# gargatik/Seamless-Through-Breaking-Rethinking-Image-Stitching-for-Optimal-Alignment

Measured on AMD Instinct MI355X. Metric: stitched image-pairs/s at 512x512, higher is better.
Workload: dtype f32 (decoder contractions, PatchEmbed's third conv and the C = 128 block tails: exact 3xbf16 split of both operands, 6 products on the bf16 matrix cores, fp32 accumulate -- error vs fp64 0.83x the fp32 MFMA chain's; everything else fp32); 1 GPU; UDIS-D-shaped 512x512 pairs, batch=1, FlowHomoAdpater.forward(type=test_eval); launch=hipGraph replay, pairs_in_flight=3

## Files before the change

seamless-through-breaking-rethinking-image-stitching-for-optimal-alignment_amd/csrc/gemm_split3.h:

```cpp
#pragma once
#include "gemm_common.h"

__global__ __launch_bounds__(256) void split3_pack_kernel(const float* __restrict__ x, __bf16* __restrict__ planes, long long rows, int C,
                                                          long long ldx, long long plane_stride, long long chunk_rows) {
    const long long idx = (long long)blockIdx.x * 256 + threadIdx.x;
    const int groups = C >> 3;
    if (idx >= rows * groups) return;
    const int g4 = (int)(idx & 3);
    const long long t = idx >> 2;
    const long long row = t % rows;
    const int chunk = (int)(t / rows);
    const float4 v0 = *reinterpret_cast<const float4*>(x + row * ldx + chunk * 32 + g4 * 8);
    const float4 v1 = *reinterpret_cast<const float4*>(x + row * ldx + chunk * 32 + g4 * 8 + 4);
    const float v[8] = {v0.x, v0.y, v0.z, v0.w, v1.x, v1.y, v1.z, v1.w};
    bf16x8 h, m, l;
#pragma unroll
    for (int e = 0; e < 8; ++e) {
        __bf16 a, b, c;
        st_split3(v[e], a, b, c);
        h[e] = a; m[e] = b; l[e] = c;
    }
    const long long o = ((long long)chunk * chunk_rows + row) * 32 + g4 * 8;
    *reinterpret_cast<bf16x8*>(planes + o) = h;
    *reinterpret_cast<bf16x8*>(planes + plane_stride + o) = m;
    *reinterpret_cast<bf16x8*>(planes + 2 * plane_stride + o) = l;
}

template <int WM, int WN, int TM, int TN, int STAGES, int KPAR = 1>
__device__ __forceinline__ void conv_gemm_split3_body(const st_gemm_desc& d, const int block_id) {
    static_assert(WM * WN == 4, "4 consumer waves per K half (+ 4 loader waves)");
    static_assert(KPAR == 1 || KPAR == 2, "one or two consumer groups");
    constexpr int BM = WM * TM * 32, BN = WN * TN * 32, ROWS = BM + BN;
    constexpr int PLANE_B = ROWS * 64, STAGE_B = 3 * PLANE_B;
    constexpr int GA = BM / 16, GB = BN / 16;
    static_assert((3 * GA) % 4 == 0 && (3 * GB) % 4 == 0, "pieces divide among the 4 loader waves");
    constexpr int PA = 3 * GA / 4, PB = 3 * GB / 4, PPW = PA + PB;
    static_assert((STAGES - 1) * PPW <= 63 && STAGES >= 3 && STAGES <= 4, "vmcnt immediate");
    extern __shared__ __attribute__((aligned(1024))) float smem[];
    char* const sm = reinterpret_cast<char*>(smem);

    const int tid = threadIdx.x;
    const int lane = tid & 63, wave = __builtin_amdgcn_readfirstlane(tid >> 6);
    const int split = d.split_k > 1 ? d.split_k : 1;
    const int bz = split > 1 ? 0 : blockIdx.z;
    const int kz = split > 1 ? blockIdx.z : 0;

    const int ntm = (d.M + BM - 1) / BM, ntn = (d.N + BN - 1) / BN;
    const int nwg = ntm * ntn;
    int bid = block_id;
    {
        const int q = nwg >> 3, r = nwg & 7, xcd = bid & 7, idx = bid >> 3;
        bid = (xcd < r ? xcd * (q + 1) : r * (q + 1) + (xcd - r) * q) + idx;
    }
    const int tile_n = bid % ntn, tile_m = bid / ntn;
    const int m0 = tile_m * BM, n0 = tile_n * BN;

    const int nkt_all = d.K / 32;
    const int per = (nkt_all + split - 1) / split;
    const int kt0 = kz * per;
    const int ntiles = min(nkt_all, kt0 + per) - kt0;

    if (wave >= 4 * KPAR) {
        const int lw = wave - 4 * KPAR;
        const char* A = reinterpret_cast<const char*>(d.a) + (size_t)bz * d.batch_stride_a * 2;
        const char* A2 = d.a2 ? reinterpret_cast<const char*>(d.a2) + (size_t)bz * d.batch_stride_a * 2 : A;
        const char* Wt = reinterpret_cast<const char*>(d.w) + (size_t)bz * d.batch_stride_w * 2;
        const i32x4 rsrcA = make_rsrc(A, d.a_bytes), rsrcA2 = make_rsrc(A2, d.a_bytes), rsrcW = make_rsrc(Wt, d.w_bytes);
        const int a2c = d.a2 ? d.a2_channels : 0;
        const unsigned lds0 = (unsigned)(size_t)(__attribute__((address_space(3))) char*)sm;
        const unsigned a_plane_b = (unsigned)(d.a_plane_stride * 2), w_plane_b = (unsigned)(d.w_plane_stride * 2);
        const unsigned a_chunk_b = (unsigned)(d.a_rows * 64), w_chunk_b = (unsigned)(d.w_rows * 64);

        int a_row[PA], a_iy0[PA], a_ix0[PA];
        unsigned a_c[PA], voffA[PA], voffB[PB], ldsA[PA], ldsB[PB];
#pragma unroll
        for (int i = 0; i < PA; ++i) {
            const int q = lw * PA + i, plane = q / GA, rg = q % GA;
            const int r = 16 * rg + (lane >> 2), c = (lane & 3) ^ ((r >> 2) & 3);
            const int m = min(m0 + r, d.M - 1);
            const int hw = d.Ho * d.Wo;
            const int b = m / hw, rr = m - b * hw;
            const int oy = rr / d.Wo, ox = rr - oy * d.Wo;
            a_iy0[i] = oy * d.sh - d.ph; a_ix0[i] = ox * d.sw - d.pw;
            a_row[i] = (b * d.H + a_iy0[i]) * d.W + a_ix0[i];
            a_c[i] = (unsigned)plane * a_plane_b + (unsigned)c * 16u;
            ldsA[i] = __builtin_amdgcn_readfirstlane(lds0 + (unsigned)(plane * PLANE_B + rg * 1024));
        }
#pragma unroll
        for (int i = 0; i < PB; ++i) {
            const int q = lw * PB + i, plane = q / GB, rg = q % GB;
            const int r = 16 * rg + (lane >> 2), c = (lane & 3) ^ ((r >> 2) & 3);
            voffB[i] = (unsigned)plane * w_plane_b + (unsigned)min(n0 + r, d.N - 1) * 64u + (unsigned)c * 16u;
            ldsB[i] = __builtin_amdgcn_readfirstlane(lds0 + (unsigned)(plane * PLANE_B + BM * 64 + rg * 1024));
        }
        int i_c0, i_ky, i_kx;
        {
            const int k = kt0 * 32, tap = k / d.Cin;
            i_c0 = k - tap * d.Cin; i_ky = tap / d.kw; i_kx = tap - i_ky * d.kw;
        }
        unsigned soffA = (unsigned)(i_c0 >> 5) * a_chunk_b, soffB = (unsigned)kt0 * w_chunk_b;
        auto set_tap = [&]() {
            const int ty = i_ky * (d.dh > 1 ? d.dh : 1), tx = i_kx * (d.dw > 1 ? d.dw : 1);
            const int tapoff = ty * d.W + tx;
#pragma unroll
            for (int i = 0; i < PA; ++i) {
                const bool ok = (unsigned)(a_iy0[i] + ty) < (unsigned)d.H && (unsigned)(a_ix0[i] + tx) < (unsigned)d.W;
                voffA[i] = ok ? a_c[i] + (unsigned)(a_row[i] + tapoff) * 64u : ST_OOB;
            }
        };
        set_tap();
        auto issue_tile = [&](int stage) {
            const unsigned so = (unsigned)(stage * STAGE_B);
            const bool second = i_c0 < a2c;
#pragma unroll
            for (int i = 0; i < PA; ++i) lds_dma16(second ? rsrcA2 : rsrcA, ldsA[i] + so, voffA[i], soffA);
#pragma unroll
            for (int i = 0; i < PB; ++i) lds_dma16(rsrcW, ldsB[i] + so, voffB[i], soffB);
            soffB += w_chunk_b; soffA += a_chunk_b;
            i_c0 += 32;
            if (i_c0 >= d.Cin) {
                i_c0 = 0; soffA = 0;
                if (++i_kx == d.kw) { i_kx = 0; ++i_ky; }
                set_tap();
            }
        };
        auto wait_tiles = [&](int tiles) {
            if (tiles >= 3) asm volatile("s_waitcnt vmcnt(%0)" ::"n"(3 * PPW) : "memory");
            else if (tiles == 2) asm volatile("s_waitcnt vmcnt(%0)" ::"n"(2 * PPW) : "memory");
            else if (tiles == 1) asm volatile("s_waitcnt vmcnt(%0)" ::"n"(PPW) : "memory");
            else asm volatile("s_waitcnt vmcnt(0)" ::: "memory");
        };
        for (int t = 0; t < STAGES && t < ntiles; ++t) issue_tile(t);
        wait_tiles(min(STAGES - 1, ntiles - 1));
        asm volatile("s_barrier" ::: "memory");
        int stage = 0;
        for (int t = 0; t + 1 < ntiles; ++t) {
            wait_tiles(min(STAGES - 2, ntiles - 2 - t));
            asm volatile("s_barrier" ::: "memory");
            if (t + STAGES < ntiles) issue_tile(stage);
            stage = stage == STAGES - 1 ? 0 : stage + 1;
        }
        return;
    }

    float* __restrict__ C = d.c + (size_t)bz * d.batch_stride_c;
    const int grp = KPAR == 2 ? wave >> 2 : 0, cw = KPAR == 2 ? wave & 3 : wave;
    const int wm = cw / WN, wn = cw % WN;
    const int li = lane & 31, lh = lane >> 5;

    f32x16 acc[TM][TN], tot[TM][TN];
#pragma unroll
    for (int i = 0; i < TM; ++i)
#pragma unroll
        for (int j = 0; j < TN; ++j)
#pragma unroll
            for (int r = 0; r < 16; ++r) { acc[i][j][r] = 0.f; tot[i][j][r] = 0.f; }
    constexpr int KBLK = 8;

    const char* pa[2];
    const char* pb[2];
#pragma unroll
    for (int j = 0; j < 2; ++j) {
        const int ch = (2 * j + lh) ^ ((li >> 2) & 3);
        pa[j] = sm + (wm * TM * 32 + li) * 64 + ch * 16;
        pb[j] = sm + (BM + wn * TN * 32 + li) * 64 + ch * 16;
    }
    if constexpr (KPAR == 2) {
        bf16x8 ga[2][3][TM], gb[2][3][TN];
        const int chg = (2 * grp + lh) ^ ((li >> 2) & 3);
        const char* const qa = sm + (wm * TM * 32 + li) * 64 + chg * 16;
        const char* const qb = sm + (BM + wn * TN * 32 + li) * 64 + chg * 16;
        auto kread = [&](int nbuf, int nstage, int set) {
            const int ra = set == 0 ? 2 : set == 1 ? 0 : 1, rb = set == 0 ? 0 : set == 1 ? 2 : 1;
#pragma unroll
            for (int r = 0; r < TM; ++r) ga[nbuf][ra][r] = *reinterpret_cast<const bf16x8*>(qa + nstage * STAGE_B + ra * PLANE_B + r * 2048);
#pragma unroll
            for (int r = 0; r < TN; ++r) gb[nbuf][rb][r] = *reinterpret_cast<const bf16x8*>(qb + nstage * STAGE_B + rb * PLANE_B + r * 2048);
        };
        auto kprod = [&](int buf, int nbuf, int p, int q, int nstage, int set) {
            const int ra = set == 0 ? 2 : set == 1 ? 0 : 1, rb = set == 0 ? 0 : set == 1 ? 2 : 1;
            constexpr int NM = TM * TN, NR = TM + TN;
            int issued = 0;
#pragma unroll
            for (int i = 0; i < TM; ++i)
#pragma unroll
                for (int jn = 0; jn < TN; ++jn) {
                    acc[i][jn] = __builtin_amdgcn_mfma_f32_32x32x16_bf16(ga[buf][p][i], gb[buf][q][jn], acc[i][jn], 0, 0, 0);
                    if (set >= 0) {
                        const int upto = ((i * TN + jn + 1) * NR + NM - 1) / NM;
#pragma unroll
                        for (int r = 0; r < NR; ++r)
                            if (r >= issued && r < upto) {
                                if (r < TM) ga[nbuf][ra][r] = *reinterpret_cast<const bf16x8*>(qa + nstage * STAGE_B + ra * PLANE_B + r * 2048);
                                else gb[nbuf][rb][r - TM] = *reinterpret_cast<const bf16x8*>(qb + nstage * STAGE_B + rb * PLANE_B + (r - TM) * 2048);
                            }
                        issued = upto;
                    }
                    __builtin_amdgcn_sched_barrier(0);
                }
        };
        constexpr bool EPI_AHEAD2 = TM * TN == 1;
        EpiOperands<TM, TN> eop2;
        if (EPI_AHEAD2 && grp == 0) {
            gemm_epilogue_consts<TM, TN>(d, eop2, n0, wn, li, split);
            gemm_epilogue_load<TM, TN>(d, eop2, m0, n0, wm, wn, li, lh, split);
            __builtin_amdgcn_sched_barrier(0);
        }
        asm volatile("s_barrier" ::: "memory");
        kread(0, 0, 0); kread(0, 0, 1); kread(0, 0, 2);
        __builtin_amdgcn_sched_barrier(0);
        auto kstep = [&](auto more_c, int buf, int nbuf, int s, int t, bool more_rt) {
            constexpr bool MORE = decltype(more_c)::value;
            if (MORE || more_rt) {
                asm volatile("s_waitcnt lgkmcnt(0)\n\ts_barrier" ::: "memory");
                kprod(buf, nbuf, 2, 0, (s + 1) % STAGES, 0); kprod(buf, nbuf, 0, 2, (s + 1) % STAGES, 1); kprod(buf, nbuf, 1, 1, (s + 1) % STAGES, 2);
            } else {
                kprod(buf, nbuf, 2, 0, 0, -1); kprod(buf, nbuf, 0, 2, 0, -1); kprod(buf, nbuf, 1, 1, 0, -1);
            }
            kprod(buf, nbuf, 1, 0, 0, -1); kprod(buf, nbuf, 0, 1, 0, -1); kprod(buf, nbuf, 0, 0, 0, -1);
            if ((t & (KBLK - 1)) == KBLK - 1 && (MORE || more_rt)) {
#pragma unroll
                for (int i = 0; i < TM; ++i)
#pragma unroll
                    for (int j = 0; j < TN; ++j) {
                        tot[i][j] = tot[i][j] + acc[i][j];
#pragma unroll
                        for (int r = 0; r < 16; ++r) acc[i][j][r] = 0.f;
                    }
                __builtin_amdgcn_sched_barrier(0);
            }
        };
        static_assert(STAGES % 2 == 0, "the fragment buffers alternate with the steps: an even ring keeps (stage, buffer) literal in the unrolled turn");
        int tb = 0;
        for (; tb + STAGES < ntiles; tb += STAGES) {
#pragma unroll
            for (int s = 0; s < STAGES; ++s) kstep(st_true{}, s & 1, (s & 1) ^ 1, s, tb + s, true);
        }
#pragma unroll
        for (int s = 0; s < STAGES; ++s)
            if (tb + s < ntiles) kstep(st_false{}, s & 1, (s & 1) ^ 1, s, tb + s, tb + s + 1 < ntiles);
        if (ntiles > KBLK) {
#pragma unroll
            for (int i = 0; i < TM; ++i)
#pragma unroll
                for (int j = 0; j < TN; ++j) acc[i][j] = acc[i][j] + tot[i][j];
        }
        asm volatile("s_waitcnt lgkmcnt(0)\n\ts_barrier" ::: "memory");
        float* const red = reinterpret_cast<float*>(sm) + (size_t)cw * (TM * TN * 16 * 64) + lane;
        if (grp == 1) {
#pragma unroll
            for (int i = 0; i < TM; ++i)
#pragma unroll
                for (int j = 0; j < TN; ++j)
#pragma unroll
                    for (int r = 0; r < 16; ++r) red[((i * TN + j) * 16 + r) * 64] = acc[i][j][r];
        }
        __syncthreads();
        if (grp == 1) return;
#pragma unroll
        for (int i = 0; i < TM; ++i)
#pragma unroll
            for (int j = 0; j < TN; ++j)
#pragma unroll
                for (int r = 0; r < 16; ++r) acc[i][j][r] += red[((i * TN + j) * 16 + r) * 64];
        if (EPI_AHEAD2) gemm_epilogue_store<TM, TN, false, false>(d, C, acc, eop2, m0, n0, wm, wn, li, lh, split, kz);
        else gemm_tile_epilogue<TM, TN>(d, C, acc, m0, n0, wm, wn, li, lh, split, kz);
        return;
    }
    bf16x8 fa[2][3][TM], fb[2][3][TN];
    auto prod = [&](int buf, int p, int q, int nbuf, int nstage, int nj, int set) {
        const int ra = set == 0 ? 2 : set == 1 ? 0 : 1, rb = set == 0 ? 0 : set == 1 ? 2 : 1;
        constexpr int NM = TM * TN, NR = TM + TN;
        int issued = 0;
#pragma unroll
        for (int i = 0; i < TM; ++i)
#pragma unroll
            for (int jn = 0; jn < TN; ++jn) {
                acc[i][jn] = __builtin_amdgcn_mfma_f32_32x32x16_bf16(fa[buf][p][i], fb[buf][q][jn], acc[i][jn], 0, 0, 0);
                if (set >= 0) {
                    const int upto = ((i * TN + jn + 1) * NR + NM - 1) / NM;
#pragma unroll
                    for (int r = 0; r < NR; ++r)
                        if (r >= issued && r < upto) {
                            if (r < TM) fa[nbuf][ra][r] = *reinterpret_cast<const bf16x8*>(pa[nj] + nstage * STAGE_B + ra * PLANE_B + r * 2048);
                            else fb[nbuf][rb][r - TM] = *reinterpret_cast<const bf16x8*>(pb[nj] + nstage * STAGE_B + rb * PLANE_B + (r - TM) * 2048);
                        }
                    issued = upto;
                }
                __builtin_amdgcn_sched_barrier(0);
            }
    };
    auto read_set = [&](int nbuf, int nstage, int nj, int set) {
        const int ra = set == 0 ? 2 : set == 1 ? 0 : 1, rb = set == 0 ? 0 : set == 1 ? 2 : 1;
#pragma unroll
        for (int r = 0; r < TM; ++r) fa[nbuf][ra][r] = *reinterpret_cast<const bf16x8*>(pa[nj] + nstage * STAGE_B + ra * PLANE_B + r * 2048);
#pragma unroll
        for (int r = 0; r < TN; ++r) fb[nbuf][rb][r] = *reinterpret_cast<const bf16x8*>(pb[nj] + nstage * STAGE_B + rb * PLANE_B + r * 2048);
    };

    constexpr bool EPI_AHEAD = TM * TN == 1;
    EpiOperands<TM, TN> eop;
    if (EPI_AHEAD) {
        gemm_epilogue_consts<TM, TN>(d, eop, n0, wn, li, split);
        gemm_epilogue_load<TM, TN>(d, eop, m0, n0, wm, wn, li, lh, split);
        __builtin_amdgcn_sched_barrier(0);
    }

    asm volatile("s_barrier" ::: "memory");
    read_set(0, 0, 0, 0); read_set(0, 0, 0, 1); read_set(0, 0, 0, 2);
    __builtin_amdgcn_sched_barrier(0);
    auto tile_body = [&](auto more_c, int s, int t, bool more_rt) {
        constexpr bool MORE = decltype(more_c)::value;
        prod(0, 2, 0, 1, s, 1, 0); prod(0, 0, 2, 1, s, 1, 1); prod(0, 1, 1, 1, s, 1, 2);
        prod(0, 1, 0, 0, 0, 0, -1); prod(0, 0, 1, 0, 0, 0, -1); prod(0, 0, 0, 0, 0, 0, -1);
        if (MORE || more_rt) {
            asm volatile("s_waitcnt lgkmcnt(0)\n\ts_barrier" ::: "memory");
            prod(1, 2, 0, 0, (s + 1) % STAGES, 0, 0); prod(1, 0, 2, 0, (s + 1) % STAGES, 0, 1); prod(1, 1, 1, 0, (s + 1) % STAGES, 0, 2);
        } else {
            prod(1, 2, 0, 0, 0, 0, -1); prod(1, 0, 2, 0, 0, 0, -1); prod(1, 1, 1, 0, 0, 0, -1);
        }
        prod(1, 1, 0, 0, 0, 0, -1); prod(1, 0, 1, 0, 0, 0, -1); prod(1, 0, 0, 0, 0, 0, -1);
        if ((t & (KBLK - 1)) == KBLK - 1 && (MORE || more_rt)) {
#pragma unroll
            for (int i = 0; i < TM; ++i)
#pragma unroll
                for (int j = 0; j < TN; ++j) {
                    tot[i][j] = tot[i][j] + acc[i][j];
#pragma unroll
                    for (int r = 0; r < 16; ++r) acc[i][j][r] = 0.f;
                }
            __builtin_amdgcn_sched_barrier(0);
        }
    };
    int tb = 0;
    for (; tb + STAGES < ntiles; tb += STAGES) {
#pragma unroll
        for (int s = 0; s < STAGES; ++s) tile_body(st_true{}, s, tb + s, true);
    }
#pragma unroll
    for (int s = 0; s < STAGES; ++s)
        if (tb + s < ntiles) tile_body(st_false{}, s, tb + s, tb + s + 1 < ntiles);
    if (ntiles > KBLK) {
#pragma unroll
        for (int i = 0; i < TM; ++i)
#pragma unroll
            for (int j = 0; j < TN; ++j) acc[i][j] = acc[i][j] + tot[i][j];
    }
    if (EPI_AHEAD) gemm_epilogue_store<TM, TN, false, false>(d, C, acc, eop, m0, n0, wm, wn, li, lh, split, kz);
    else gemm_tile_epilogue<TM, TN>(d, C, acc, m0, n0, wm, wn, li, lh, split, kz);
}

template <bool CT>
__device__ __forceinline__ void conv_gemm_split3_persist_body(const st_gemm_desc& d) {
    constexpr int BM = 64, BN = 64, ROWS = 128, STAGES = 3, WN = 2;
    constexpr int PLANE_B = ROWS * 64, STAGE_B = 3 * PLANE_B, GA = 4, GB = 4, PA = 3, PB = 3, PPW = 6;
    extern __shared__ __attribute__((aligned(1024))) float smem[];
    char* const sm = reinterpret_cast<char*>(smem);
    const int tid = threadIdx.x;
    const int lane = tid & 63, wave = __builtin_amdgcn_readfirstlane(tid >> 6);
    const int bz = blockIdx.z;
    const int ntm = (d.M + BM - 1) / BM, ntn = (d.N + BN - 1) / BN, ntl = ntm * ntn;
    const int G = (int)gridDim.x, w = (int)blockIdx.x;
    const int nmine = (ntl - w + G - 1) / G;
    const int nkt = d.K / 32;
    const int total = nmine * nkt;

    if (wave >= 4) {
        const int lw = wave - 4;
        const char* A = reinterpret_cast<const char*>(d.a) + (size_t)bz * d.batch_stride_a * 2;
        const char* Wt = reinterpret_cast<const char*>(d.w) + (size_t)bz * d.batch_stride_w * 2;
        const i32x4 rsrcA = make_rsrc(A, d.a_bytes), rsrcW = make_rsrc(Wt, d.w_bytes);
        const unsigned lds0 = (unsigned)(size_t)(__attribute__((address_space(3))) char*)sm;
        const unsigned a_plane_b = (unsigned)(d.a_plane_stride * 2), w_plane_b = (unsigned)(d.w_plane_stride * 2);
        const unsigned a_chunk_b = (unsigned)(d.a_rows * 64), w_chunk_b = (unsigned)(d.w_rows * 64);
        int a_row[PA], a_iy0[PA], a_ix0[PA];
        unsigned a_c[PA], voffA[PA], voffB[PB], ldsA[PA], ldsB[PB];
#pragma unroll
        for (int i = 0; i < PA; ++i) {
            const int q = lw * PA + i, plane = q / GA, rg = q % GA;
            ldsA[i] = __builtin_amdgcn_readfirstlane(lds0 + (unsigned)(plane * PLANE_B + rg * 1024));
        }
#pragma unroll
        for (int i = 0; i < PB; ++i) {
            const int q = lw * PB + i, plane = q / GB, rg = q % GB;
            ldsB[i] = __builtin_amdgcn_readfirstlane(lds0 + (unsigned)(plane * PLANE_B + BM * 64 + rg * 1024));
        }
        int i_c0 = 0, i_ky = 0, i_kx = 0, i_kt = 0, i_tile = w;
        unsigned soffA = 0, soffB = 0;
        auto set_tap = [&]() {
            const int ty = i_ky * (d.dh > 1 ? d.dh : 1), tx = i_kx * (d.dw > 1 ? d.dw : 1);
            const int tapoff = ty * d.W + tx;
#pragma unroll
            for (int i = 0; i < PA; ++i) {
                const bool ok = (unsigned)(a_iy0[i] + ty) < (unsigned)d.H && (unsigned)(a_ix0[i] + tx) < (unsigned)d.W;
                voffA[i] = ok ? a_c[i] + (unsigned)(a_row[i] + tapoff) * 64u : ST_OOB;
            }
        };
        auto set_tile = [&](int idx) {
            const int m0 = (idx / ntn) * BM, n0 = (idx % ntn) * BN;
#pragma unroll
            for (int i = 0; i < PA; ++i) {
                const int q = lw * PA + i, plane = q / GA, rg = q % GA;
                const int r = 16 * rg + (lane >> 2), c = (lane & 3) ^ ((r >> 2) & 3);
                const int m = min(m0 + r, d.M - 1);
                const int hw = d.Ho * d.Wo;
                const int b = m / hw, rr = m - b * hw;
                const int oy = rr / d.Wo, ox = rr - oy * d.Wo;
                a_iy0[i] = oy * d.sh - d.ph; a_ix0[i] = ox * d.sw - d.pw;
                a_row[i] = (b * d.H + a_iy0[i]) * d.W + a_ix0[i];
                a_c[i] = (unsigned)plane * a_plane_b + (unsigned)c * 16u;
            }
#pragma unroll
            for (int i = 0; i < PB; ++i) {
                const int q = lw * PB + i, plane = q / GB, rg = q % GB;
                const int r = 16 * rg + (lane >> 2), c = (lane & 3) ^ ((r >> 2) & 3);
                voffB[i] = (unsigned)plane * w_plane_b + (unsigned)min(n0 + r, d.N - 1) * 64u + (unsigned)c * 16u;
            }
            i_c0 = 0; i_ky = 0; i_kx = 0; i_kt = 0; soffA = 0; soffB = 0;
            set_tap();
        };
        set_tile(i_tile);
        auto issue_step = [&](int stage) {
            const unsigned so = (unsigned)(stage * STAGE_B);
            const unsigned sa = __builtin_amdgcn_readfirstlane(soffA), sb = __builtin_amdgcn_readfirstlane(soffB);
#pragma unroll
            for (int i = 0; i < PA; ++i) lds_dma16(rsrcA, ldsA[i] + so, voffA[i], sa);
#pragma unroll
            for (int i = 0; i < PB; ++i) lds_dma16(rsrcW, ldsB[i] + so, voffB[i], sb);
            if (++i_kt == nkt) { i_tile += G; if (i_tile < ntl) set_tile(i_tile); return; }
            soffB += w_chunk_b; soffA += a_chunk_b;
            i_c0 += 32;
            if (i_c0 >= d.Cin) {
                i_c0 = 0; soffA = 0;
                if (++i_kx == d.kw) { i_kx = 0; ++i_ky; }
                set_tap();
            }
        };
        auto wait_tiles = [&](int tiles) {
            if (tiles >= 2) asm volatile("s_waitcnt vmcnt(%0)" ::"n"(2 * PPW) : "memory");
            else if (tiles == 1) asm volatile("s_waitcnt vmcnt(%0)" ::"n"(PPW) : "memory");
            else asm volatile("s_waitcnt vmcnt(0)" ::: "memory");
        };
        for (int t = 0; t < STAGES && t < total; ++t) issue_step(t);
        wait_tiles(min(STAGES - 1, total - 1));
        asm volatile("s_barrier" ::: "memory");
        int stage = 0;
        for (int t = 0; t + 1 < total; ++t) {
            wait_tiles(min(STAGES - 2, total - 2 - t));
            asm volatile("s_barrier" ::: "memory");
            if (t + STAGES < total) issue_step(stage);
            stage = stage == STAGES - 1 ? 0 : stage + 1;
        }
        return;
    }

    float* __restrict__ C = d.c + (size_t)bz * d.batch_stride_c;
    const int wm = wave / WN, wn = wave % WN;
    const int li = lane & 31, lh = lane >> 5;
    f32x16 acc[1][1], tot;
    constexpr int KBLK = 8;
    unsigned offA[2], offB[2];
#pragma unroll
    for (int j = 0; j < 2; ++j) {
        const int ch = (2 * j + lh) ^ ((li >> 2) & 3);
        offA[j] = (unsigned)((wm * 32 + li) * 64 + ch * 16);
        offB[j] = (unsigned)((BM + wn * 32 + li) * 64 + ch * 16);
    }
    bf16x8 fa[2][3], fb[2][3];
    auto read_set = [&](int nbuf, int so, int nj, int set) {
        const int ra = set == 0 ? 2 : set == 1 ? 0 : 1, rb = set == 0 ? 0 : set == 1 ? 2 : 1;
        fa[nbuf][ra] = *reinterpret_cast<const bf16x8*>(sm + so + ra * PLANE_B + offA[nj]);
        fb[nbuf][rb] = *reinterpret_cast<const bf16x8*>(sm + so + rb * PLANE_B + offB[nj]);
    };
    auto prod = [&](int buf, int p, int q, int nbuf, int so, int nj, int set) {
        acc[0][0] = __builtin_amdgcn_mfma_f32_32x32x16_bf16(fa[buf][p], fb[buf][q], acc[0][0], 0, 0, 0);
        if (set >= 0) read_set(nbuf, so, nj, set);
        __builtin_amdgcn_sched_barrier(0);
    };
    asm volatile("s_barrier" ::: "memory");
    read_set(0, 0, 0, 0); read_set(0, 0, 0, 1); read_set(0, 0, 0, 2);
    __builtin_amdgcn_sched_barrier(0);
    auto step_body = [&](auto more_c, int stage, int kt) {
        constexpr bool MORE = decltype(more_c)::value;
        const int so = stage * STAGE_B, sn = (stage == STAGES - 1 ? 0 : stage + 1) * STAGE_B;
        prod(0, 2, 0, 1, so, 1, 0); prod(0, 0, 2, 1, so, 1, 1); prod(0, 1, 1, 1, so, 1, 2);
        prod(0, 1, 0, 0, 0, 0, -1); prod(0, 0, 1, 0, 0, 0, -1); prod(0, 0, 0, 0, 0, 0, -1);
        if (MORE) {
            asm volatile("s_waitcnt lgkmcnt(0)\n\ts_barrier" ::: "memory");
            prod(1, 2, 0, 0, sn, 0, 0); prod(1, 0, 2, 0, sn, 0, 1); prod(1, 1, 1, 0, sn, 0, 2);
        } else {
            prod(1, 2, 0, 0, 0, 0, -1); prod(1, 0, 2, 0, 0, 0, -1); prod(1, 1, 1, 0, 0, 0, -1);
        }
        prod(1, 1, 0, 0, 0, 0, -1); prod(1, 0, 1, 0, 0, 0, -1); prod(1, 0, 0, 0, 0, 0, -1);
        if ((kt & (KBLK - 1)) == KBLK - 1 && kt + 1 < nkt) {
            tot = tot + acc[0][0];
#pragma unroll
            for (int r = 0; r < 16; ++r) acc[0][0][r] = 0.f;
            __builtin_amdgcn_sched_barrier(0);
        }
    };
    int stage = 0;
    for (int ti = 0; ti < nmine; ++ti) {
        const int idx = w + ti * G;
        const int m0 = (idx / ntn) * BM, n0 = (idx % ntn) * BN;
#pragma unroll
        for (int r = 0; r < 16; ++r) { acc[0][0][r] = 0.f; tot[r] = 0.f; }
        const int nsteps = ti == nmine - 1 ? nkt - 1 : nkt;
        for (int kt = 0; kt < nsteps; ++kt) {
            step_body(st_true{}, stage, kt);
            stage = stage == STAGES - 1 ? 0 : stage + 1;
        }
        if (ti == nmine - 1) step_body(st_false{}, stage, nkt - 1);
        if (nkt > KBLK) acc[0][0] = acc[0][0] + tot;
        {
            EpiOperands<1, 1> eop;
            gemm_epilogue_consts<1, 1>(d, eop, n0, wn, li, 1);
            gemm_epilogue_load<1, 1>(d, eop, m0, n0, wm, wn, li, lh, 1);
            gemm_epilogue_store<1, 1, false, CT>(d, C, acc, eop, m0, n0, wm, wn, li, lh, 1, 0);
        }
    }
}

template <bool CT>
__global__ __launch_bounds__(512, 4) void conv_gemm_split3_persist_kernel(const st_gemm_desc d) {
    conv_gemm_split3_persist_body<CT>(d);
}

template <int WM, int WN, int TM, int TN, int STAGES>
__global__ __launch_bounds__(512) void conv_gemm_split3_kernel(const st_gemm_desc d) {
    conv_gemm_split3_body<WM, WN, TM, TN, STAGES>(d, (int)blockIdx.x);
}
template <int WM, int WN, int TM, int TN, int STAGES>
__global__ __launch_bounds__(768, 1) void conv_gemm_split3_kpar_kernel(const st_gemm_desc d) {
    conv_gemm_split3_body<WM, WN, TM, TN, STAGES, 2>(d, (int)blockIdx.x);
}

template <int STAGES>
__global__ __launch_bounds__(512, 4) void conv_gemm_split3_kernel64(const st_gemm_desc d) {
    conv_gemm_split3_body<2, 2, 1, 1, STAGES>(d, (int)blockIdx.x);
}

template <int WM, int WN, int TM, int TN, int STAGES>
__global__ __launch_bounds__(512, 4) void conv_gemm_split3_pair_kernel(const st_gemm_pair_args g) {
    const bool second = (int)blockIdx.x >= g.tiles0;
    conv_gemm_split3_body<WM, WN, TM, TN, STAGES>(second ? g.d[1] : g.d[0], second ? (int)blockIdx.x - g.tiles0 : (int)blockIdx.x);
}
```

Baseline: 98.85 pairs/s.

## Use 16x16x32 bf16 MFMA path with new LDS swizzle in split3 conv GEMMs

After: 99.62 pairs/s, median of 6. About the same (+0.8%).

```diff
diff --git a/seamless-through-breaking-rethinking-image-stitching-for-optimal-alignment_amd/csrc/gemm_split3.h b/seamless-through-breaking-rethinking-image-stitching-for-optimal-alignment_amd/csrc/gemm_split3.h
--- a/seamless-through-breaking-rethinking-image-stitching-for-optimal-alignment_amd/csrc/gemm_split3.h
+++ b/seamless-through-breaking-rethinking-image-stitching-for-optimal-alignment_amd/csrc/gemm_split3.h
@@ -1,5 +1,7 @@
 #pragma once
 #include "gemm_common.h"
+
+typedef float f32x4 __attribute__((ext_vector_type(4)));
 
 __global__ __launch_bounds__(256) void split3_pack_kernel(const float* __restrict__ x, __bf16* __restrict__ planes, long long rows, int C,
                                                           long long ldx, long long plane_stride, long long chunk_rows) {
@@ -26,7 +28,13 @@
     *reinterpret_cast<bf16x8*>(planes + 2 * plane_stride + o) = l;
 }
 
-template <int WM, int WN, int TM, int TN, int STAGES, int KPAR = 1>
+#ifndef ST_SPLIT3_MFMA16
+#define ST_SPLIT3_MFMA16 7
+#endif
+template <bool S16>
+__device__ __forceinline__ int split3_swz(int r) { return S16 ? (4 - (r >> 2)) & 3 : (r >> 2) & 3; }
+
+template <int WM, int WN, int TM, int TN, int STAGES, int KPAR = 1, bool S16 = false>
 __device__ __forceinline__ void conv_gemm_split3_body(const st_gemm_desc& d, const int block_id) {
     static_assert(WM * WN == 4, "4 consumer waves per K half (+ 4 loader waves)");
     static_assert(KPAR == 1 || KPAR == 2, "one or two consumer groups");
@@ -76,7 +84,7 @@
 #pragma unroll
         for (int i = 0; i < PA; ++i) {
             const int q = lw * PA + i, plane = q / GA, rg = q % GA;
-            const int r = 16 * rg + (lane >> 2), c = (lane & 3) ^ ((r >> 2) & 3);
+            const int r = 16 * rg + (lane >> 2), c = (lane & 3) ^ split3_swz<S16>(r);
             const int m = min(m0 + r, d.M - 1);
             const int hw = d.Ho * d.Wo;
             const int b = m / hw, rr = m - b * hw;
@@ -89,7 +97,7 @@
 #pragma unroll
         for (int i = 0; i < PB; ++i) {
             const int q = lw * PB + i, plane = q / GB, rg = q % GB;
-            const int r = 16 * rg + (lane >> 2), c = (lane & 3) ^ ((r >> 2) & 3);
+            const int r = 16 * rg + (lane >> 2), c = (lane & 3) ^ split3_swz<S16>(r);
             voffB[i] = (unsigned)plane * w_plane_b + (unsigned)min(n0 + r, d.N - 1) * 64u + (unsigned)c * 16u;
             ldsB[i] = __builtin_amdgcn_readfirstlane(lds0 + (unsigned)(plane * PLANE_B + BM * 64 + rg * 1024));
         }
@@ -164,6 +172,174 @@
         const int ch = (2 * j + lh) ^ ((li >> 2) & 3);
         pa[j] = sm + (wm * TM * 32 + li) * 64 + ch * 16;
         pb[j] = sm + (BM + wn * TN * 32 + li) * 64 + ch * 16;
+    }
+    if constexpr (S16) {
+        constexpr int HA = 2 * TM, HB = 2 * TN, NM = HA * HB;
+        const int r16 = lane & 15, slot = (lane >> 4) ^ split3_swz<true>(r16);
+        const char* const qa = sm + grp * STAGE_B + (wm * TM * 32 + r16) * 64 + slot * 16;
+        const char* const qb = sm + grp * STAGE_B + (BM + wn * TN * 32 + r16) * 64 + slot * 16;
+        f32x4 a4[HA][HB], t4[HA][HB];
+#pragma unroll
+        for (int i = 0; i < HA; ++i)
+#pragma unroll
+            for (int j = 0; j < HB; ++j)
+#pragma unroll
+                for (int r = 0; r < 4; ++r) { a4[i][j][r] = 0.f; t4[i][j][r] = 0.f; }
+        bf16x8 ga[2][3][HA], gb[2][3][HB];
+        auto rdA = [&](int buf, int p, int nstage, int h) {
+            ga[p == 0 ? buf : 0][p][h] = *reinterpret_cast<const bf16x8*>(qa + nstage * STAGE_B + p * PLANE_B + h * 1024);
+        };
+        auto rdB = [&](int buf, int p, int nstage, int h) {
+            gb[p == 0 ? buf : 0][p][h] = *reinterpret_cast<const bf16x8*>(qb + nstage * STAGE_B + p * PLANE_B + h * 1024);
+        };
+        auto read_tile = [&](int buf, int nstage) {
+#pragma unroll
+            for (int p = 2; p >= 0; --p) {
+#pragma unroll
+                for (int h = 0; h < HA; ++h) rdA(buf, p, nstage, h);
+#pragma unroll
+                for (int h = 0; h < HB; ++h) rdB(buf, p, nstage, h);
+            }
+        };
+        auto prod16 = [&](int buf, int p, int q, int nstage, int ra, int rb) {
+            const int NR = (ra >= 0 ? HA : 0) + (rb >= 0 ? HB : 0), na = ra >= 0 ? HA : 0;
+            int issued = 0;
+#pragma unroll
+            for (int i = 0; i < HA; ++i)
+#pragma unroll
+                for (int j = 0; j < HB; ++j) {
+                    a4[i][j] = __builtin_amdgcn_mfma_f32_16x16x32_bf16(ga[p == 0 ? buf : 0][p][i], gb[q == 0 ? buf : 0][q][j], a4[i][j], 0, 0, 0);
+                    const int upto = ((i * HB + j + 1) * NR + NM - 1) / NM;
+#pragma unroll
+                    for (int r = 0; r < HA + HB; ++r)
+                        if (r >= issued && r < upto) {
+                            if (r < na) rdA(buf ^ 1, ra, nstage, r);
+                            else rdB(buf ^ 1, rb, nstage, r - na);
+                        }
+                    issued = upto;
+                    __builtin_amdgcn_sched_barrier(0);
+                }
+        };
+        auto fold16 = [&]() {
+#pragma unroll
+            for (int i = 0; i < HA; ++i)
+#pragma unroll
+                for (int j = 0; j < HB; ++j) {
+                    t4[i][j] = t4[i][j] + a4[i][j];
+#pragma unroll
+                    for (int r = 0; r < 4; ++r) a4[i][j][r] = 0.f;
+                }
+            __builtin_amdgcn_sched_barrier(0);
+        };
+        constexpr bool EPI_AHEAD16 = TM * TN == 1;
+        EpiOperands<TM, TN> eop16;
+        if (EPI_AHEAD16 && grp == 0) {
+            gemm_epilogue_consts<TM, TN>(d, eop16, n0, wn, li, split);
+            gemm_epilogue_load<TM, TN>(d, eop16, m0, n0, wm, wn, li, lh, split);
+            __builtin_amdgcn_sched_barrier(0);
+        }
+        asm volatile("s_barrier" ::: "memory");
+        if constexpr (KPAR == 2) {
+            static_assert(KPAR == 1 || STAGES == 4, "a group's tiles alternate between two stages of a 4-deep ring");
+            if (grp == 1 && ntiles > 1) asm volatile("s_barrier" ::: "memory");
+            if (grp < ntiles) read_tile(0, 0);
+            __builtin_amdgcn_sched_barrier(0);
+            auto kstep16 = [&](auto more_c, int buf, int rs, int t) {
+                constexpr bool MORE = decltype(more_c)::value;
+                const bool b0 = MORE || t + 1 < ntiles, b1 = MORE || t + 2 < ntiles;
+                const int ns = rs ^ 2;
+                prod16(buf, 2, 0, 0, -1, -1);
+                if (b0) asm volatile("s_waitcnt lgkmcnt(0)\n\ts_barrier" ::: "memory");
+                prod16(buf, 0, 2, 0, -1, -1); prod16(buf, 1, 1, 0, -1, -1);
+                if (b1) {
+                    asm volatile("s_barrier" ::: "memory");
+                    prod16(buf, 1, 0, ns, 2, 2);
+                    prod16(buf, 0, 1, ns, 1, 0);
+                    prod16(buf, 0, 0, ns, 0, 1);
+                    if ((t & (KBLK - 1)) >= KBLK - 2) fold16();
+                } else {
+                    prod16(buf, 1, 0, 0, -1, -1); prod16(buf, 0, 1, 0, -1, -1); prod16(buf, 0, 0, 0, -1, -1);
+                }
+            };
+            int t = grp;
+            for (; t + 4 < ntiles; t += 4) { kstep16(st_true{}, 0, 0, t); kstep16(st_true{}, 1, 2, t + 2); }
+            if (t < ntiles) kstep16(st_false{}, 0, 0, t);
+            if (t + 2 < ntiles) kstep16(st_false{}, 1, 2, t + 2);
+        } else {
+            read_tile(0, 0);
+            __builtin_amdgcn_sched_barrier(0);
+            auto step16 = [&](auto more_c, int buf, int s, int t, bool more_rt) {
+                constexpr bool MORE = decltype(more_c)::value;
+                const int ns = (s + 1) % STAGES;
+                prod16(buf, 2, 0, 0, -1, -1);
+                if (MORE || more_rt) {
+                    asm volatile("s_waitcnt lgkmcnt(0)\n\ts_barrier" ::: "memory");
+                    prod16(buf, 0, 2, ns, 2, 0);
+                    prod16(buf, 1, 1, ns, 0, 2);
+                    prod16(buf, 1, 0, ns, -1, -1);
+                    prod16(buf, 0, 1, ns, 1, -1);
+                    prod16(buf, 0, 0, ns, -1, 1);
+                    if ((t & (KBLK - 1)) == KBLK - 1) fold16();
+                } else {
+                    prod16(buf, 0, 2, 0, -1, -1); prod16(buf, 1, 1, 0, -1, -1); prod16(buf, 1, 0, 0, -1, -1);
+                    prod16(buf, 0, 1, 0, -1, -1); prod16(buf, 0, 0, 0, -1, -1);
+                }
+            };
+            constexpr int TURN = STAGES % 2 ? 2 * STAGES : STAGES;
+            int tb = 0;
+            for (; tb + TURN < ntiles; tb += TURN) {
+#pragma unroll
+                for (int s = 0; s < TURN; ++s) step16(st_true{}, s & 1, s % STAGES, tb + s, true);
+            }
+#pragma unroll
+            for (int s = 0; s < TURN; ++s)
+                if (tb + s < ntiles) step16(st_false{}, s & 1, s % STAGES, tb + s, tb + s + 1 < ntiles);
+        }
+        if (ntiles > KBLK) {
+#pragma unroll
+            for (int i = 0; i < HA; ++i)
+#pragma unroll
+                for (int j = 0; j < HB; ++j) a4[i][j] = a4[i][j] + t4[i][j];
+        }
+        if constexpr (KPAR == 2) {
+            asm volatile("s_waitcnt lgkmcnt(0)\n\ts_barrier" ::: "memory");
+            float* const red = reinterpret_cast<float*>(sm) + (size_t)cw * (TM * TN * 16 * 64) + lane;
+            if (grp == 1) {
+#pragma unroll
+                for (int i = 0; i < HA; ++i)
+#pragma unroll
+                    for (int j = 0; j < HB; ++j)
+#pragma unroll
+                        for (int r = 0; r < 4; ++r) red[((i * HB + j) * 4 + r) * 64] = a4[i][j][r];
+            }
+            __syncthreads();
+            if (grp == 1) return;
+#pragma unroll
+            for (int i = 0; i < HA; ++i)
+#pragma unroll
+                for (int j = 0; j < HB; ++j)
+#pragma unroll
+                    for (int r = 0; r < 4; ++r) a4[i][j][r] += red[((i * HB + j) * 4 + r) * 64];
+        }
+        const bool hn = (lane >> 4) & 1;
+#pragma unroll
+        for (int i = 0; i < TM; ++i)
+#pragma unroll
+            for (int j = 0; j < TN; ++j)
+#pragma unroll
+                for (int q = 0; q < 4; ++q) {
+                    const int src = ((lane & 15) + 16 * ((2 * q + lh) & 3)) * 4;
+#pragma unroll
+                    for (int r = 0; r < 4; ++r) {
+                        const float x0 = a4[2 * i + (q >> 1)][2 * j][r], x1 = a4[2 * i + (q >> 1)][2 * j + 1][r];
+                        const int v0 = __builtin_amdgcn_ds_bpermute(src, __float_as_int(x0));
+                        const int v1 = __builtin_amdgcn_ds_bpermute(src, __float_as_int(x1));
+                        acc[i][j][4 * q + r] = __int_as_float(hn ? v1 : v0);
+                    }
+                }
+        if (EPI_AHEAD16) gemm_epilogue_store<TM, TN, false, false>(d, C, acc, eop16, m0, n0, wm, wn, li, lh, split, kz);
+        else gemm_tile_epilogue<TM, TN>(d, C, acc, m0, n0, wm, wn, li, lh, split, kz);
+        return;
     }
     if constexpr (KPAR == 2) {
         bf16x8 ga[2][3][TM], gb[2][3][TN];
@@ -528,20 +704,20 @@
 
 template <int WM, int WN, int TM, int TN, int STAGES>
 __global__ __launch_bounds__(512) void conv_gemm_split3_kernel(const st_gemm_desc d) {
-    conv_gemm_split3_body<WM, WN, TM, TN, STAGES>(d, (int)blockIdx.x);
+    conv_gemm_split3_body<WM, WN, TM, TN, STAGES, 1, (ST_SPLIT3_MFMA16 & 1) != 0 && TM * TN < 4>(d, (int)blockIdx.x);
 }
 template <int WM, int WN, int TM, int TN, int STAGES>
 __global__ __launch_bounds__(768, 1) void conv_gemm_split3_kpar_kernel(const st_gemm_desc d) {
-    conv_gemm_split3_body<WM, WN, TM, TN, STAGES, 2>(d, (int)blockIdx.x);
+    conv_gemm_split3_body<WM, WN, TM, TN, STAGES, 2, (ST_SPLIT3_MFMA16 & 4) != 0 && TM * TN == 1>(d, (int)blockIdx.x);
 }
 
 template <int STAGES>
 __global__ __launch_bounds__(512, 4) void conv_gemm_split3_kernel64(const st_gemm_desc d) {
-    conv_gemm_split3_body<2, 2, 1, 1, STAGES>(d, (int)blockIdx.x);
+    conv_gemm_split3_body<2, 2, 1, 1, STAGES, 1, (ST_SPLIT3_MFMA16 & 2) != 0>(d, (int)blockIdx.x);
 }
 
 template <int WM, int WN, int TM, int TN, int STAGES>
 __global__ __launch_bounds__(512, 4) void conv_gemm_split3_pair_kernel(const st_gemm_pair_args g) {
     const bool second = (int)blockIdx.x >= g.tiles0;
-    conv_gemm_split3_body<WM, WN, TM, TN, STAGES>(second ? g.d[1] : g.d[0], second ? (int)blockIdx.x - g.tiles0 : (int)blockIdx.x);
+    conv_gemm_split3_body<WM, WN, TM, TN, STAGES, 1, (ST_SPLIT3_MFMA16 & 2) != 0>(second ? g.d[1] : g.d[0], second ? (int)blockIdx.x - g.tiles0 : (int)blockIdx.x);
 }
```
